# BOpermanis/SP-SLAM

Measured on AMD Instinct MI355X. Metric: RGB-D frames/sec (track+planes+poseOpt) at 640x480; ATE vs CPU ref, higher is better.
Workload: dtype u8+f32+f64

## Files before the change

### include/spslam_gpu.h

```cpp
#ifndef SPSLAM_GPU_H
#define SPSLAM_GPU_H

#include <stddef.h>
#include <stdint.h>

#ifdef __cplusplus
extern "C" {
#endif

#define SPSLAM_OK 0
#define SPSLAM_ERR_ARG (-1)
#define SPSLAM_ERR_CAPACITY (-2)
#define SPSLAM_ERR_HIP (-3)
#define SPSLAM_ERR_NOT_READY (-4)

typedef struct spslam_ctx spslam_ctx;

typedef struct spslam_keypoint {
    float x, y;
    float size;
    float angle;
    float response;
    int32_t octave;
    int32_t class_id;
// ... 232 lines not shown
int spslam_supposed_debug(spslam_ctx* ctx, int frame, int plane, spslam_line_candidate* cand, int* n_cand,
                          int32_t* idx, int idx_cap);

int spslam_planes_debug(spslam_ctx* ctx, int frame, int what, void* out, int* n_points);

int spslam_debug_plane_labels(spslam_ctx* ctx, int keep);

typedef struct spslam_plane_launch_shape {
    int32_t seg_maps_in_lds;
    int32_t seg_positions;
    int32_t wave_count;
    int32_t one_workgroup;
    int32_t barrier_rows;
} spslam_plane_launch_shape;
int spslam_debug_plane_launch_shape(spslam_ctx* ctx, int n_frames, spslam_plane_launch_shape* shape);

int spslam_debug_plane_not_seen(spslam_ctx* ctx, const float* planes, int n_planes, const float* coefs, int n_coefs,
                                int* not_seen);

int spslam_debug_libm64(spslam_ctx* ctx, int kind, const double* a, const double* b, int n, double* out);

int spslam_debug_pose_spin_cap(spslam_ctx* ctx, int cap);

int spslam_debug_force_solve_failures(spslam_ctx* ctx, unsigned trial_mask);

#define SPSLAM_GRID_COLS 64
#define SPSLAM_GRID_ROWS 48

typedef struct spslam_frame_params {
    float fx, fy, cx, cy;
// ... 495 lines not shown
```

### sp-slam_amd/csrc/capi_planes.cpp

```cpp
#include "capi_ctx.h"

#include <cmath>
#include <cstring>
#include <random>
#include <string>

namespace {

hipError_t configure_supposed(spslam_ctx* c, const spslam_plane_params* p) {
    const PlaneGeom& g = c->pg;
    SuppParams& sp = c->sp;
    sp.line_ratio = p->line_ratio;
    const double T = (double)p->line_distance_threshold * (double)p->line_distance_threshold;
    float f = (float)T;
    while ((double)f >= T && f > 0.f) f = std::nextafter(f, 0.f);
    while ((double)std::nextafter(f, 1.f) < T) f = std::nextafter(f, 1.f);
    sp.sqr_th_f = f;
    const bool nob = p->image_bounds[0] == 0.f && p->image_bounds[1] == 0.f && p->image_bounds[2] == 0.f &&
                     p->image_bounds[3] == 0.f;
    sp.min_x = nob ? 0.f : p->image_bounds[0];
    sp.max_x = nob ? (float)p->width : p->image_bounds[1];
    sp.min_y = nob ? 0.f : p->image_bounds[2];
    sp.max_y = nob ? (float)p->height : p->image_bounds[3];
    sp.supp_cap = kMaxSuppPerFrame;
    sp.line_cap = g.contour_cap;
    int ns = 0;
    for (float v = -0.25f; v < 0.25f; v = (float)((double)v + 0.01)) {
        if (ns >= kMaxPatchSteps) return hipErrorInvalidValue;
        sp.steps[ns++] = v;
    }
    sp.n_steps = ns;
    const size_t F = (size_t)c->p.max_batch, CC = (size_t)g.contour_cap;
    SuppBuffers& b = c->sb;
    const size_t bytes = (size_t)kSuppRndTable * 4 +
                         F * kMaxPlanesPerFrame * kMaxLinesPerBoundary * sizeof(LineCand) +
                         F * kMaxPlanesPerFrame * sizeof(int) + F * CC * (4 + 16 + 4 + 1) +
                         F * kMaxPlanesPerFrame * 8 * sizeof(long long) + 9 * 256;
    hipError_t e = c->d_supp_scratch.alloc(bytes);
    if (e != hipSuccess) return e;
    uint8_t* q = c->d_supp_scratch;
    auto carve = [&](size_t n) { uint8_t* r = q; q += (n + 255) / 256 * 256; return r; };
    b.rnd = (const uint32_t*)carve((size_t)kSuppRndTable * 4);
    b.cand = (LineCand*)carve(F * kMaxPlanesPerFrame * kMaxLinesPerBoundary * sizeof(LineCand));
    b.n_cand = (int*)carve(F * kMaxPlanesPerFrame * sizeof(int));
    b.line_idx = (int32_t*)carve(F * CC * 4);
    b.big = (float4*)carve(F * CC * 16);
    b.big_sh = (int*)carve(F * CC * 4);
    b.big_flag = (uint8_t*)carve(F * CC);
    b.prof = (long long*)carve(F * kMaxPlanesPerFrame * 8 * sizeof(long long));
    e = hipMemset(b.prof, 0, F * kMaxPlanesPerFrame * 8 * sizeof(long long));
    if (e != hipSuccess) return e;
    std::vector<uint32_t> tab(kSuppRndTable);
    std::mt19937 mt(12345u);
    for (auto& v : tab) v = (uint32_t)mt() >> 1;
    e = hipMemcpy((void*)b.rnd, tab.data(), tab.size() * 4, hipMemcpyHostToDevice);
    if (e != hipSuccess) return e;
    const size_t patch = (size_t)sp.n_steps * sp.n_steps;
    if ((e = c->d_supp1.alloc(sp.supp_cap * sizeof(spslam_supposed_plane))) != hipSuccess) return e;
    if ((e = c->d_supp_cnt1.alloc(16)) != hipSuccess) return e;
    if ((e = c->d_line1.alloc(CC * 4)) != hipSuccess) return e;
    return c->d_patch1.alloc(sp.supp_cap * patch * 12);
}

int plane_status_flags(long long word, int epoch) { return (word >> 8) == epoch ? (int)(word & 0xFF) : 0; }

}

extern "C" {

int spslam_planes_configure(spslam_ctx* c, const spslam_plane_params* p) {
// ... 15 lines not shown
    if (plane_launch_shape(g, 1, nullptr) != hipSuccess)
        return fail(c, SPSLAM_ERR_ARG, "no kernel instance takes the organized cloud%s",
                    g.W > 512 ? ": wider than 512 columns" : ": past the segmentation's LDS or index budget");
    g.fx = p->fx; g.fy = p->fy; g.cx = p->cx; g.cy = p->cy;
    g.min_size = p->min_size;
    g.ang_cos = std::cos((float)(0.017453 * p->angle_threshold));
    g.dist_th = p->distance_threshold;
    g.inlier_cap = g.N;
    g.contour_cap = 4 * g.N;
    c->pg = g;
    const long long N = g.N, F = c->p.max_batch, IWH = (long long)(g.W + 1) * (g.H + 1);
    PlaneBuffers& b = c->pb;
    c->planes_ready = false;
    c->plane_last_frames = c->supp_last_frames = 0;
    c->plane_cloud[0] = c->plane_cloud[1] = nullptr;
    c->sb = SuppBuffers{};
    const int keep_labels = b.keep_labels;
    b = PlaneBuffers{};
    b.keep_labels = keep_labels;
    const long long SH = wave_size(g.W, g.H);
    b.cloud_fs = 3 * N; b.wave_fs = SH; b.dist_fs = N; b.integral_fs = 6 * (IWH + g.W + 1); b.normal_fs = 3 * N; b.pd_fs = N;
    b.labels_fs = N; b.work_fs = 4 * N; b.grown_fs = N; b.maps_fs = 2 * N;
    const size_t bytes = F * (sizeof(float) * (2 * b.cloud_fs + b.wave_fs + b.dist_fs + b.normal_fs + b.pd_fs) +
                              sizeof(double) * b.integral_fs + sizeof(uint32_t) * b.labels_fs +
                              sizeof(int) * (b.work_fs + b.grown_fs) + b.maps_fs + 16 * sizeof(long long)) + 8192;
    HIP_CHECK(c, c->d_plane_scratch.alloc(bytes));
    uint8_t* q = c->d_plane_scratch;
    auto carve = [&](size_t n) { uint8_t* r = q; q += (n + 255) / 256 * 256; return r; };
    b.integral = (double*)carve(F * b.integral_fs * sizeof(double));
    c->plane_cloud[0] = (float*)carve(F * b.cloud_fs * 4);
    c->plane_cloud[1] = (float*)carve(F * b.cloud_fs * 4);
// ... 264 lines not shown
        return rc;
    HIP_CHECK(c, plane_not_seen_debug_launch(st.slot<float>(0), n_planes, st.slot<float>(1), n_coefs,
                                             st.slot<int>(2), c->stream));
    HIP_CHECK(c, hipMemcpyAsync(not_seen, st.slot<int>(2), (size_t)n_coefs * 4, hipMemcpyDeviceToHost, c->stream));
    if (int rc = st.close()) return rc;
    HIP_CHECK(c, hipStreamSynchronize(c->stream));
    return SPSLAM_OK;
}

int spslam_debug_plane_labels(spslam_ctx* c, int keep) {
    if (!c) return SPSLAM_ERR_ARG;
    c->pb.keep_labels = keep ? 1 : 0;
    return SPSLAM_OK;
}

int spslam_supposed_debug(spslam_ctx* c, int frame, int plane, spslam_line_candidate* cand, int* n_cand,
                          int32_t* idx, int idx_cap) {
    static_assert(sizeof(spslam_line_candidate) == sizeof(LineCand), "candidate layout");
    if (!c || !cand || !n_cand) return SPSLAM_ERR_ARG;
    if (frame < 0 || frame >= c->supp_last_frames || plane < 0 || plane >= kMaxPlanesPerFrame)
        return fail(c, SPSLAM_ERR_NOT_READY, "no supposed-plane data for that frame%s", "");
    HIP_CHECK(c, hipSetDevice(c->device));
    HIP_CHECK(c, hipDeviceSynchronize());
    int nc = 0;
    HIP_CHECK(c, hipMemcpy(&nc, c->sb.n_cand + frame * kMaxPlanesPerFrame + plane, sizeof(int), hipMemcpyDeviceToHost));
    nc = std::min(std::max(nc, 0), kMaxLinesPerBoundary);
    LineCand lc[kMaxLinesPerBoundary];
    if (nc)
        HIP_CHECK(c, hipMemcpy(lc, c->sb.cand + ((size_t)frame * kMaxPlanesPerFrame + plane) * kMaxLinesPerBoundary,
                               nc * sizeof(LineCand), hipMemcpyDeviceToHost));
// ... 61 lines not shown
```

### sp-slam_amd/csrc/supposed_kernels.hip

```cpp
#include "pcl_eigen33.h"
#include "plane_not_seen.h"
#include "supposed_launch.h"
#include "wave_ops.h"

namespace spslam {
namespace supp {

using namespace pcl_eigen;

constexpr int kThreads = 256, kWaves = 4;
constexpr int kMaxWaves = 8;
constexpr int kBatch = 64;
constexpr int kLdsPts = 2048;
constexpr int kMaxTrials = 1001;

#ifdef SPSLAM_SUPP_PROF
#define SUPP_CLK() ((long long)__builtin_amdgcn_s_memrealtime())
#define SUPP_T(k) do { if (t == 0) { const long long c_ = SUPP_CLK(); pr[k] += c_ - pt; pt = c_; } } while (0)
#else
#define SUPP_T(k) do { } while (0)
#endif

struct Shared {
    int s0[kBatch], s1[kBatch], cnt[kBatch];
    int nb, fail, done, have;
    int iterations, best, best_s0, best_s1;
    double k;
    float line[6];
    float acc[9];
    int red[kMaxWaves];
    int n_inl, flags;
    int s0x[kBatch], s1x[kBatch], nbb[2], failb[2];
};

template <int NT>
__device__ int block_sum(int v, Shared& S) {
    const int lane = threadIdx.x & 63, wave = threadIdx.x >> 6;
    v = wave_sum(v);
    __syncthreads();
    if (lane == 0) S.red[wave] = v;
    __syncthreads();
    int s = 0;
#pragma unroll
    for (int w = 0; w < NT / 64; w++) s += S.red[w];
    return s;
}

// ... 103 lines not shown
}

template <int NT>
__device__ int select_within(const float* coef, const float4* Q, uint8_t* flag, int n, float thr, Shared& S) {
    float lp[3] = {coef[0], coef[1], coef[2]}, ld[3] = {coef[3], coef[4], coef[5]};
    normalize4(ld);
    int c = 0;
    for (int i = threadIdx.x; i < n; i += NT) {
        const bool in = line_sqd(lp, ld, Q[i]) <= thr;
        flag[i] = in;
        c += in;
    }
    return block_sum<NT>(c, S);
}

#ifndef SPSLAM_SUPP_OVERLAP
#define SPSLAM_SUPP_OVERLAP 1
#endif
#ifndef SPSLAM_SUPP_OVERLAP_ALL
#define SPSLAM_SUPP_OVERLAP_ALL 0
#endif
#ifndef SPSLAM_SUPP_MINB
#define SPSLAM_SUPP_MINB 3
#endif
template <int NT>
__global__ __launch_bounds__(NT, NT == 256 ? SPSLAM_SUPP_MINB : 1) void supp_lines_kernel(PlaneGeom g, PlaneBuffers pb, SuppParams sp,
                                                              SuppBuffers sb, const float* __restrict__ depth,
                                                              long long depth_fs, int depth_stride,
                                                              const spslam_plane* __restrict__ planes,
                                                              const int* __restrict__ plane_counts,
                                                              const int32_t* __restrict__ contours) {
    __shared__ float4 Qs[kLdsPts];
    __shared__ int shs[kLdsPts];
    __shared__ uint8_t flags_s[kLdsPts];
#ifdef SPSLAM_MEASURE_SKIP_SUPP
    if (g.W > 0) return;
#endif
    __shared__ Shared S;
    constexpr bool kOverlap = SPSLAM_SUPP_OVERLAP && (NT == 512 || SPSLAM_SUPP_OVERLAP_ALL);
    const int f = blockIdx.x, t = threadIdx.x, lane = t & 63, wave = t >> 6;
    const int np = min(plane_counts[f], kMaxPlanesPerFrame);
    const spslam_plane* P = planes + (size_t)f * kMaxPlanesPerFrame;
    const int32_t* con = contours + (size_t)f * g.contour_cap;
    const float* X = pb.cloud + f * pb.cloud_fs;
    const float* Y = X + g.N;
    const float* Z = X + 2 * g.N;
    const Cam K{g.fx, g.fy, g.cx, g.cy, sp.min_x, sp.max_x, sp.min_y, sp.max_y, g.w, g.h, depth_stride};
    const float* D = depth + f * depth_fs;
    const float thr = sp.sqr_th_f;
    for (int q = blockIdx.y; q < np; q += gridDim.y) {
        LineCand* C = sb.cand + ((size_t)f * kMaxPlanesPerFrame + q) * kMaxLinesPerBoundary;
        const int bsize = P[q].n_contour, coff = P[q].contour_offset;
        if (bsize < 50) {
            if (t == 0) sb.n_cand[f * kMaxPlanesPerFrame + q] = 0;
            continue;
        }
        const bool in_lds = bsize <= kLdsPts;
        int32_t* lidx = sb.line_idx + (size_t)f * g.contour_cap + coff;
        auto boundary = [&](float4* Q, int* sh, uint8_t* flag) __attribute__((always_inline)) -> int {
#ifdef SPSLAM_SUPP_PROF
        long long pr[8] = {0, 0, 0, 0, 0, 0, 0, 0}, pt = SUPP_CLK();
#endif
        for (int i = t; i < bsize; i += NT) {
            const int ci = con[coff + i];
            Q[i] = make_float4(X[ci], Y[ci], Z[ci], __int_as_float(ci));
        }
        __syncthreads();
        SUPP_T(0);
        int n = bsize, used = 0, ncand = 0;
        for (int j = 0; j < kMaxLinesPerBoundary; j++) {
            if (t == 0) {
                S.iterations = 0; S.best = -2147483647; S.k = 1.0; S.have = 0; S.done = n < 2;
            }
            if constexpr (kOverlap) {
                if (t < kBatch) S.cnt[t] = 0;
            }
            for (int i = t; i < n; i += NT) sh[i] = i;
            __syncthreads();
            const double one_over_n = 1.0 / (double)n, log_prob = log(1.0 - 0.99);
            int r0 = 0, r1 = 1;
            uint32_t pos = 0;
            int bp0 = 0, bp1 = 0, qh = 0, qn = 0;
            uint64_t gmask = 0;
            uint32_t rnext = wave == 0 ? sb.rnd[lane] : 0u;
            if constexpr (!kOverlap) {
                while (!S.done) {
                    if (wave == 0) {
                        const int it0 = S.iterations;
                        int nb = 0, chk = 0;
                        bool fail = false;
                        while (nb < kBatch && it0 + nb < kMaxTrials) {
                            if (qh == qn) {
                                const uint32_t r = rnext;
                                const uint32_t jv = (lane & 1) ? 1u + r % (uint32_t)(n - 1) : r % (uint32_t)n;
                                pos += 64;
                                rnext = sb.rnd[pos + lane];
    #pragma unroll 4
                                for (int c = 0; c < 32; c++) {
                                    const int j0 = __builtin_amdgcn_readlane((int)jv, 2 * c), j1 = __builtin_amdgcn_readlane((int)jv, 2 * c + 1);
                                    const int i0 = j0 > 1 ? j0 : 0, i1 = j1 > 1 ? j1 : 1;
                                    const int x0 = sh[i0], x1 = sh[i1];
                                    const int a0 = r0, b0 = r1;
                                    const int r1m = j0 == 1 ? a0 : b0;
                                    sh[i0] = a0;
                                    sh[i1] = r1m;
                                    r0 = j0 > 1 ? x0 : (j0 == 1 ? b0 : a0);
                                    r1 = j1 > 1 ? (j1 == j0 ? a0 : x1) : r1m;
                                    bp0 = lane == c ? r0 : bp0;
                                    bp1 = lane == c ? r1 : bp1;
                                }
                                bool good = false;
                                if (lane < 32) {
                                    const float4 a = Q[bp0], b = Q[bp1];
                                    good = a.x != b.x && a.y != b.y && a.z != b.z;
                                }
                                gmask = __ballot(good);
                                qh = 0;
                                qn = 32;
                            }
                            const uint64_t m = gmask & (~0ull << qh) & 0xFFFFFFFFull;
                            if (m == 0) {
                                chk += qn - qh;
                                qh = qn;
                                if (chk >= 1000) { fail = true; break; }
                                continue;
                            }
                            const int gi = __ffsll((unsigned long long)m) - 1;
                            if (chk + (gi - qh) >= 1000) { fail = true; break; }
                            const int s0v = __builtin_amdgcn_readlane(bp0, gi), s1v = __builtin_amdgcn_readlane(bp1, gi);
                            if (lane == 0) { S.s0[nb] = s0v; S.s1[nb] = s1v; }
                            nb++;
                            chk = 0;
                            qh = gi + 1;
                        }
                        if (lane == 0) { S.nb = nb; S.fail = fail; }
                    }
                    __syncthreads();
                    SUPP_T(1);
                    const int nb = S.nb;
                    {
                        constexpr int NW = NT / 64;
                        const int c = wave * (kBatch / NW) + lane / NW, qq = lane % NW;
                        int cnt = 0;
                        if (c < nb) {
                            float L[6];
                            line_from_samples(Q[S.s0[c]], Q[S.s1[c]], L);
                            float ld[3] = {L[3], L[4], L[5]};
                            normalize4(ld);
    #pragma unroll 1
                            for (int i = qq; i < n; i += NW) cnt += line_sqd(L, ld, Q[i]) <= thr;
                        }
    #pragma unroll
                        for (int o = 1; o < NW; o <<= 1) cnt += __shfl_xor(cnt, o);
                        if (qq == 0 && c < nb) S.cnt[c] = cnt;
                    }
                    __syncthreads();
                    SUPP_T(2);
                    if (wave == 0) {
                        const int it0 = S.iterations, best0 = S.best;
                        const double k0 = S.k;
                        const bool act = lane < nb;
                        const int cn = act ? S.cnt[lane] : INT_MIN;
                        int pm = cn, lr;
    #pragma unroll
                        for (int off = 1; off < 64; off <<= 1) {
                            const int y = __shfl_up(pm, off);
                            if (lane >= off) pm = max(pm, y);
                        }
                        int ex = __shfl_up(pm, 1);
                        if (lane == 0) ex = INT_MIN;
                        const bool rec = act && cn > max(ex, best0);
                        double kc = 0.0;
                        if (rec) {
                            const double w = (double)cn * one_over_n;
                            double pno = 1.0 - w * w;
                            pno = fmax(DBL_EPSILON, pno);
                            pno = fmin(1.0 - DBL_EPSILON, pno);
                            kc = log_prob / log(pno);
                        }
                        lr = rec ? lane : -1;
    #pragma unroll
                        for (int off = 1; off < 64; off <<= 1) {
                            const int y = __shfl_up(lr, off);
                            if (lane >= off) lr = max(lr, y);
                        }
                        int lre = __shfl_up(lr, 1);
                        if (lane == 0) lre = -1;
                        const double kb_rec = __shfl(kc, lre < 0 ? 0 : lre);
                        const double kb = lre < 0 ? k0 : kb_rec;
                        const uint64_t m1 = __ballot(act && !((double)(it0 + lane) < kb));
                        const int stop1 = m1 ? __ffsll((unsigned long long)m1) - 1 : 64;
                        const int stop2 = (kMaxTrials - 1) - it0;
                        int proc, it;
                        bool done;
                        if (stop1 < nb && stop1 <= stop2) { proc = stop1; it = it0 + stop1; done = true; }
                        else if (stop2 < nb) { proc = stop2 + 1; it = it0 + stop2 + 1; done = true; }
                        else { proc = nb; it = it0 + nb; done = false; }
                        const uint64_t rm = __ballot(rec) & (proc >= 64 ? ~0ull : ((1ull << proc) - 1ull));
                        double kf = k0;
                        if (rm) {
                            const int L = 63 - __clzll(rm);
                            kf = __shfl(kc, L);
                            if (lane == L) {
                                S.best = cn; S.best_s0 = S.s0[L]; S.best_s1 = S.s1[L]; S.have = 1; S.k = kc;
                            }
                        }
                        if (!done && (S.fail || !((double)it < kf))) done = true;
                        if (lane == 0) {
                            S.iterations = it;
                            S.done = done;
                        }
                    }
                    __syncthreads();
                    SUPP_T(3);
    #ifdef SPSLAM_SUPP_PROF
                    if (t == 0) pr[6]++;
    #endif
                }
            } else {
                auto sample = [&](int sb_, int it0) __attribute__((always_inline)) {
                    int nb = 0, chk = 0;
                    bool fail = false;
                    while (nb < kBatch && it0 + nb < kMaxTrials) {
                        if (qh == qn) {
                            const uint32_t r = rnext;
                            const uint32_t jv = (lane & 1) ? 1u + r % (uint32_t)(n - 1) : r % (uint32_t)n;
                            pos += 64;
                            rnext = sb.rnd[pos + lane];
    #pragma unroll 4
                            for (int c = 0; c < 32; c++) {
                                const int j0 = __builtin_amdgcn_readlane((int)jv, 2 * c), j1 = __builtin_amdgcn_readlane((int)jv, 2 * c + 1);
                                const int i0 = j0 > 1 ? j0 : 0, i1 = j1 > 1 ? j1 : 1;
                                const int x0 = sh[i0], x1 = sh[i1];
                                const int a0 = r0, b0 = r1;
                                const int r1m = j0 == 1 ? a0 : b0;
                                sh[i0] = a0;
                                sh[i1] = r1m;
                                r0 = j0 > 1 ? x0 : (j0 == 1 ? b0 : a0);
                                r1 = j1 > 1 ? (j1 == j0 ? a0 : x1) : r1m;
                                bp0 = lane == c ? r0 : bp0;
                                bp1 = lane == c ? r1 : bp1;
                            }
                            bool good = false;
                            if (lane < 32) {
                                const float4 a = Q[bp0], b = Q[bp1];
                                good = a.x != b.x && a.y != b.y && a.z != b.z;
                            }
                            gmask = __ballot(good);
                            qh = 0;
                            qn = 32;
                        }
                        const uint64_t m = gmask & (~0ull << qh) & 0xFFFFFFFFull;
                        if (m == 0) {
                            chk += qn - qh;
                            qh = qn;
                            if (chk >= 1000) { fail = true; break; }
                            continue;
                        }
                        const int gi = __ffsll((unsigned long long)m) - 1;
                        if (chk + (gi - qh) >= 1000) { fail = true; break; }
                        const int s0v = __builtin_amdgcn_readlane(bp0, gi), s1v = __builtin_amdgcn_readlane(bp1, gi);
                        if (lane == 0) { (sb_ ? S.s0x : S.s0)[nb] = s0v; (sb_ ? S.s1x : S.s1)[nb] = s1v; }
                        nb++;
                        chk = 0;
                        qh = gi + 1;
                    }
                    if (lane == 0) { S.nbb[sb_] = nb; S.failb[sb_] = fail; }
                };
                auto decide = [&](int sb_, int nb) __attribute__((always_inline)) {
                    const int it0 = S.iterations, best0 = S.best;
                    const double k0 = S.k;
                    const bool act = lane < nb;
                    const int cn = act ? S.cnt[lane] : INT_MIN;
                    int pm = cn, lr;
    #pragma unroll
                    for (int off = 1; off < 64; off <<= 1) {
                        const int y = __shfl_up(pm, off);
                        if (lane >= off) pm = max(pm, y);
                    }
                    int ex = __shfl_up(pm, 1);
                    if (lane == 0) ex = INT_MIN;
                    const bool rec = act && cn > max(ex, best0);
                    double kc = 0.0;
                    if (rec) {
                        const double w = (double)cn * one_over_n;
                        double pno = 1.0 - w * w;
                        pno = fmax(DBL_EPSILON, pno);
                        pno = fmin(1.0 - DBL_EPSILON, pno);
                        kc = log_prob / log(pno);
                    }
                    lr = rec ? lane : -1;
    #pragma unroll
                    for (int off = 1; off < 64; off <<= 1) {
                        const int y = __shfl_up(lr, off);
                        if (lane >= off) lr = max(lr, y);
                    }
                    int lre = __shfl_up(lr, 1);
                    if (lane == 0) lre = -1;
                    const double kb_rec = __shfl(kc, lre < 0 ? 0 : lre);
                    const double kb = lre < 0 ? k0 : kb_rec;
                    const uint64_t m1 = __ballot(act && !((double)(it0 + lane) < kb));
                    const int stop1 = m1 ? __ffsll((unsigned long long)m1) - 1 : 64;
                    const int stop2 = (kMaxTrials - 1) - it0;
                    int proc, it;
                    bool done;
                    if (stop1 < nb && stop1 <= stop2) { proc = stop1; it = it0 + stop1; done = true; }
                    else if (stop2 < nb) { proc = stop2 + 1; it = it0 + stop2 + 1; done = true; }
                    else { proc = nb; it = it0 + nb; done = false; }
                    const uint64_t rm = __ballot(rec) & (proc >= 64 ? ~0ull : ((1ull << proc) - 1ull));
                    double kf = k0;
                    if (rm) {
                        const int L = 63 - __clzll(rm);
                        kf = __shfl(kc, L);
                        if (lane == L) {
                            S.best = cn; S.best_s0 = (sb_ ? S.s0x : S.s0)[L]; S.best_s1 = (sb_ ? S.s1x : S.s1)[L];
                            S.have = 1; S.k = kc;
                        }
                    }
                    if (!done && (S.failb[sb_] || !((double)it < kf))) done = true;
                    if (lane == 0) {
                        S.iterations = it;
                        S.done = done;
                    }
                };
                if (wave == 0 && !S.done) sample(0, 0);
                __syncthreads();
                SUPP_T(1);
                int cur = 0;
                while (!S.done) {
                    const int nb = S.nbb[cur];
                    if (wave == 0) {
                        if (!S.failb[cur]) sample(cur ^ 1, S.iterations + nb);
                        else if (lane == 0) { S.nbb[cur ^ 1] = 0; S.failb[cur ^ 1] = 1; }
                    } else {
                        constexpr int LP = NT / 64 - 1;
                        const int u = t - 64, c = u / LP, qq = u - c * LP;
                        if (c < nb) {
                            float L[6];
                            line_from_samples(Q[(cur ? S.s0x : S.s0)[c]], Q[(cur ? S.s1x : S.s1)[c]], L);
                            float ld[3] = {L[3], L[4], L[5]};
                            normalize4(ld);
                            int cnt = 0;
#pragma unroll 1
                            for (int i = qq; i < n; i += LP) cnt += line_sqd(L, ld, Q[i]) <= thr;
                            atomicAdd(&S.cnt[c], cnt);
                        }
                    }
                    __syncthreads();
                    SUPP_T(2);
                    if (wave == 0) {
                        decide(cur, nb);
                        S.cnt[lane] = 0;
                    }
                    __syncthreads();
                    SUPP_T(3);
#ifdef SPSLAM_SUPP_PROF
                    if (t == 0) pr[6]++;
#endif
                    cur ^= 1;
                }
            }
            int n_inl = 0;
            if (S.have) {
                float c0[6];
                line_from_samples(Q[S.best_s0], Q[S.best_s1], c0);
                n_inl = select_within<NT>(c0, Q, flag, n, thr, S);
                if (n_inl > 2) {
                    constexpr int kG = 8;
                    if (wave == 0 && lane < 3) {
                        float s = 0.f;
                        int i = 0;
                        for (; i + kG <= n; i += kG) {
                            float v[kG];
#pragma unroll
                            for (int u = 0; u < kG; u++) {
                                const float4 p = Q[i + u];
                                v[u] = flag[i + u] ? (lane == 0 ? p.x : lane == 1 ? p.y : p.z) : 0.f;
                            }
#pragma unroll
                            for (int u = 0; u < kG; u++) s += v[u];
                        }
                        for (; i < n; i++) {
                            const float4 p = Q[i];
                            s += flag[i] ? (lane == 0 ? p.x : lane == 1 ? p.y : p.z) : 0.f;
                        }
                        S.acc[lane] = s / (float)n_inl;
                    }
                    __syncthreads();
                    if (wave == 0 && lane < 6) {
                        const float cx = S.acc[0], cy = S.acc[1], cz = S.acc[2];
                        auto term = [&](int i) __attribute__((always_inline)) {
                            const float4 p = Q[i];
                            const float x = p.x - cx, y = p.y - cy, z = p.z - cz;
                            const float a = lane == 0 ? y : lane == 1 ? y : lane == 2 ? z : lane == 3 ? x : lane == 4 ? y : z;
                            const float b = lane == 0 ? y : lane == 1 ? z : lane == 2 ? z : x;
                            return flag[i] ? a * b : 0.f;
                        };
                        float s = 0.f;
                        int i = 0;
                        for (; i + kG <= n; i += kG) {
                            float v[kG];
#pragma unroll
                            for (int u = 0; u < kG; u++) v[u] = term(i + u);
#pragma unroll
                            for (int u = 0; u < kG; u++) s += v[u];
                        }
                        for (; i < n; i++) s += term(i);
                        S.acc[3 + lane] = s;
                    }
                    __syncthreads();
                    if (t == 0) {
                        const float cov[3][3] = {{S.acc[6], S.acc[7], S.acc[8]},
                                                 {S.acc[7], S.acc[3], S.acc[4]},
                                                 {S.acc[8], S.acc[4], S.acc[5]}};
                        float ev[3];
                        line_direction(cov, ev);
                        S.line[0] = S.acc[0]; S.line[1] = S.acc[1]; S.line[2] = S.acc[2];
                        S.line[3] = ev[0]; S.line[4] = ev[1]; S.line[5] = ev[2];
                    }
                } else if (t == 0) {
                    for (int k = 0; k < 6; k++) S.line[k] = c0[k];
                }
// ... 51 lines not shown
            nonborder = block_sum<NT>(nonborder, S);
            if (t == 0) out.flags = fl | ((fl & 2) && nonborder <= n_inl / 4 ? 4 : 0);
            used += n_inl;
            n = kbase;
            __syncthreads();
            SUPP_T(5);
        }
#ifdef SPSLAM_SUPP_PROF
        if (t == 0) {
            pr[7] = bsize;
            for (int k = 0; k < 8; k++) sb.prof[((size_t)f * kMaxPlanesPerFrame + q) * 8 + k] = pr[k];
        }
#endif
            return ncand;
        };
        const int ncand = in_lds ? boundary(Qs, shs, flags_s)
                                 : boundary(sb.big + (size_t)f * g.contour_cap + coff,
                                            sb.big_sh + (size_t)f * g.contour_cap + coff,
                                            sb.big_flag + (size_t)f * g.contour_cap + coff);
        if (t == 0) sb.n_cand[f * kMaxPlanesPerFrame + q] = ncand;
        __syncthreads();
    }
}

__device__ void supposed_coef(const float* ip, const float* il, float* coef) {
    const float a = fmaf(ip[1], il[5], -(ip[2] * il[4]));
    const float b = fmaf(ip[2], il[3], -(ip[0] * il[5]));
    const float c = fmaf(ip[0], il[4], -(ip[1] * il[3]));
    const float d = fmaf(c, il[2], fmaf(a, il[0], b * il[1]));
    const float v = sqrtf(fmaf(c, c, fmaf(a, a, b * b)));
    coef[0] = a / v; coef[1] = b / v; coef[2] = c / v; coef[3] = -d / v;
    if (coef[3] < 0)
        for (int k = 0; k < 4; k++) coef[k] = -coef[k];
}
// ... 118 lines not shown
```

### sp-slam_amd/csrc/supposed_launch.h

```cpp
#pragma once
#include <hip/hip_runtime.h>

#include "../../include/spslam_gpu.h"
#include "orb_launch.h"
#include "plane_launch.h"

namespace spslam {

constexpr int kMaxLinesPerBoundary = 4;
constexpr int kSuppRndTable = 1 << 21;
constexpr int kMaxPatchSteps = 64;
constexpr int kMaxSuppPerFrame = 32;

struct LineCand {
    float line[6];
    int n_inliers;
    int iterations;
    int flags;
    int idx_off;
};

struct SuppParams {
    double line_ratio;
    float sqr_th_f;
    float min_x, max_x, min_y, max_y;
    int supp_cap;
    int line_cap;
    int n_steps;
    float steps[kMaxPatchSteps];
};

struct SuppBuffers {
    const uint32_t* rnd;
    LineCand* cand;
    int* n_cand;
    int32_t* line_idx;
    float4* big;
    int* big_sh;
    uint8_t* big_flag;
    long long* prof;
};

hipError_t supp_launch(const PlaneGeom& g, const PlaneBuffers& pb, const SuppParams& sp, const SuppBuffers& sb,
                       int n, const float* depth, long long depth_fs, int depth_stride, const spslam_plane* planes,
                       const int* plane_counts, const int32_t* contours, spslam_supposed_plane* out, int* out_counts,
                       int32_t* out_line_idx, float* out_patch, hipStream_t s, KernelTimer* timer);

hipError_t plane_not_seen_debug_launch(const float* planes, int n, const float* coefs, int m, int* out,
// ... 4 lines not shown
```

### sp-slam_amd/spslam_planes.py

```python
from __future__ import annotations

import ctypes

import numpy as np

import spslam_gpu

PLANE_DTYPE = np.dtype([("coef", "<f4", 4), ("n_inliers", "<i4"), ("inlier_offset", "<i4"), ("n_contour", "<i4"),
                        ("contour_offset", "<i4")])
assert PLANE_DTYPE.itemsize == 32


class PlaneParams(ctypes.Structure):
    _fields_ = [("cloud_dis", ctypes.c_int), ("min_size", ctypes.c_int), ("angle_threshold", ctypes.c_float),
                ("distance_threshold", ctypes.c_float), ("fx", ctypes.c_float), ("fy", ctypes.c_float),
                ("cx", ctypes.c_float), ("cy", ctypes.c_float), ("width", ctypes.c_int), ("height", ctypes.c_int),
                ("line_ratio", ctypes.c_double), ("line_distance_threshold", ctypes.c_float),
                ("image_bounds", ctypes.c_float * 4)]


SUPPOSED_DTYPE = np.dtype([("coef", "<f4", 4), ("line", "<f4", 6), ("source_plane", "<i4"), ("n_line", "<i4"),
                           ("line_offset", "<i4"), ("n_patch", "<i4"), ("patch_offset", "<i4"), ("pad", "<i4")])
assert SUPPOSED_DTYPE.itemsize == 64
LINE_CAND_DTYPE = np.dtype([("line", "<f4", 6), ("n_inliers", "<i4"), ("iterations", "<i4"), ("flags", "<i4"),
                            ("idx_offset", "<i4")])


spslam_gpu.EXPORTED += ["spslam_planes_configure", "spslam_planes_capacity", "spslam_planes_extract",
                        "spslam_planes_extract_batch_device", "spslam_planes_debug", "spslam_debug_plane_labels",
                        "spslam_supposed_capacity",
                        "spslam_planes_generate_from_boundaries",
                        "spslam_planes_generate_from_boundaries_batch_device", "spslam_supposed_debug",
                        "spslam_planes_select_cloud_set",
                        "spslam_debug_plane_not_seen", "spslam_planes_status", "spslam_debug_plane_launch_shape"]

OVER_COMPONENTS, OVER_MODELS, OVER_KEPT = 1, 2, 4


class PlaneLaunchShape(ctypes.Structure):
    _fields_ = [("seg_maps_in_lds", ctypes.c_int32), ("seg_positions", ctypes.c_int32),
                ("wave_count", ctypes.c_int32), ("one_workgroup", ctypes.c_int32), ("barrier_rows", ctypes.c_int32)]


def _bind(lib):
    vp, ip = ctypes.c_void_p, ctypes.POINTER(ctypes.c_int)
    lib.spslam_planes_configure.argtypes = [vp, ctypes.POINTER(PlaneParams)]
    lib.spslam_planes_capacity.argtypes = [vp, ip, ip, ip]
    lib.spslam_planes_extract.argtypes = [vp, vp, ctypes.c_int, ctypes.c_int, ctypes.c_int, vp, ctypes.c_int, ip, vp,
                                          vp]
# ... 77 lines not shown

    def status(self, frame=0):
        flags = ctypes.c_int(-1)
        self.ex._check(self.ex.lib.spslam_planes_status(self.ex.ctx, frame, ctypes.byref(flags)))
        return flags.value

    def launch_shape(self, n_frames=1):
        sh = PlaneLaunchShape()
        self.ex._check(self.ex.lib.spslam_debug_plane_launch_shape(self.ex.ctx, n_frames, ctypes.byref(sh)))
        return {name: int(getattr(sh, name)) for name, _ in PlaneLaunchShape._fields_}

    def keep_labels(self, on=True):
        self.ex.lib.spslam_debug_plane_labels.argtypes = [ctypes.c_void_p, ctypes.c_int]
        self.ex._check(self.ex.lib.spslam_debug_plane_labels(self.ex.ctx, int(on)))

    def debug(self, frame, what):
        N = self.W * self.H
        shape, dt = {0: ((N, 3), np.float32), 1: ((N, 3), np.float32), 2: (N, np.float32), 3: (N, np.uint32)}[what]
        out = np.zeros(shape, dt)
        n = ctypes.c_int()
        self.ex._check(self.ex.lib.spslam_planes_debug(self.ex.ctx, frame, what, out.ctypes.data, ctypes.byref(n)))
        return out

    def generate_from_boundaries(self, depth_f32: np.ndarray):
        d = np.ascontiguousarray(depth_f32, np.float32)
        out = np.zeros(self.supp_cap, SUPPOSED_DTYPE)
        lines = np.zeros(self.line_cap, np.int32)
        patch = np.zeros((self.supp_cap * self.patch_points, 3), np.float32)
        n = ctypes.c_int()
        self.ex._check(self.ex.lib.spslam_planes_generate_from_boundaries(
# ... 34 lines not shown
```

Before: 44550.

## Precompute RANSAC sample-pair table per point count and compact inliers for line refit

```diff
diff --git a/include/spslam_gpu.h b/include/spslam_gpu.h
--- a/include/spslam_gpu.h
+++ b/include/spslam_gpu.h
@@ -270,6 +270,10 @@
     int32_t barrier_rows;
 } spslam_plane_launch_shape;
 int spslam_debug_plane_launch_shape(spslam_ctx* ctx, int n_frames, spslam_plane_launch_shape* shape);
+
+int spslam_debug_supposed_table_depth(spslam_ctx* ctx, int pairs);
+
+int spslam_debug_supposed_table_row(spslam_ctx* ctx, int n, uint32_t* pairs);
 
 int spslam_debug_plane_not_seen(spslam_ctx* ctx, const float* planes, int n_planes, const float* coefs, int n_coefs,
                                 int* not_seen);
diff --git a/sp-slam_amd/csrc/capi_planes.cpp b/sp-slam_amd/csrc/capi_planes.cpp
--- a/sp-slam_amd/csrc/capi_planes.cpp
+++ b/sp-slam_amd/csrc/capi_planes.cpp
@@ -32,15 +32,17 @@
     sp.n_steps = ns;
     const size_t F = (size_t)c->p.max_batch, CC = (size_t)g.contour_cap;
     SuppBuffers& b = c->sb;
-    const size_t bytes = (size_t)kSuppRndTable * 4 +
+    const size_t n_samples = supp_sample_row(kSuppTabMaxN + 1);
+    const size_t bytes = (size_t)kSuppRndTable * 4 + n_samples * 4 +
                          F * kMaxPlanesPerFrame * kMaxLinesPerBoundary * sizeof(LineCand) +
                          F * kMaxPlanesPerFrame * sizeof(int) + F * CC * (4 + 16 + 4 + 1) +
-                         F * kMaxPlanesPerFrame * 8 * sizeof(long long) + 9 * 256;
+                         F * kMaxPlanesPerFrame * 8 * sizeof(long long) + 10 * 256;
     hipError_t e = c->d_supp_scratch.alloc(bytes);
     if (e != hipSuccess) return e;
     uint8_t* q = c->d_supp_scratch;
     auto carve = [&](size_t n) { uint8_t* r = q; q += (n + 255) / 256 * 256; return r; };
     b.rnd = (const uint32_t*)carve((size_t)kSuppRndTable * 4);
+    b.samples = (const uint32_t*)carve(n_samples * 4);
     b.cand = (LineCand*)carve(F * kMaxPlanesPerFrame * kMaxLinesPerBoundary * sizeof(LineCand));
     b.n_cand = (int*)carve(F * kMaxPlanesPerFrame * sizeof(int));
     b.line_idx = (int32_t*)carve(F * CC * 4);
@@ -54,6 +56,9 @@
     std::mt19937 mt(12345u);
     for (auto& v : tab) v = (uint32_t)mt() >> 1;
     e = hipMemcpy((void*)b.rnd, tab.data(), tab.size() * 4, hipMemcpyHostToDevice);
+    if (e != hipSuccess) return e;
+    const std::vector<uint32_t> samples = build_supp_sample_table(tab.data());
+    e = hipMemcpy((void*)b.samples, samples.data(), samples.size() * 4, hipMemcpyHostToDevice);
     if (e != hipSuccess) return e;
     const size_t patch = (size_t)sp.n_steps * sp.n_steps;
     if ((e = c->d_supp1.alloc(sp.supp_cap * sizeof(spslam_supposed_plane))) != hipSuccess) return e;
@@ -99,7 +104,9 @@
     c->planes_ready = false;
     c->plane_last_frames = c->supp_last_frames = 0;
     c->plane_cloud[0] = c->plane_cloud[1] = nullptr;
+    const int tab_depth = c->sb.tab_depth;
     c->sb = SuppBuffers{};
+    c->sb.tab_depth = tab_depth;
     const int keep_labels = b.keep_labels;
     b = PlaneBuffers{};
     b.keep_labels = keep_labels;
@@ -394,6 +401,20 @@
     return SPSLAM_OK;
 }
 
+int spslam_debug_supposed_table_depth(spslam_ctx* c, int pairs) {
+    if (!c || pairs < 0 || pairs > kSuppTabPairs) return SPSLAM_ERR_ARG;
+    c->sb.tab_depth = pairs;
+    return SPSLAM_OK;
+}
+
+int spslam_debug_supposed_table_row(spslam_ctx* c, int n, uint32_t* pairs) {
+    if (!c || !pairs || n < kSuppTabMinN || n > kSuppTabMaxN) return SPSLAM_ERR_ARG;
+    if (!c->planes_ready) return fail(c, SPSLAM_ERR_NOT_READY, "spslam_planes_configure not called%s", "");
+    HIP_CHECK(c, hipSetDevice(c->device));
+    HIP_CHECK(c, hipMemcpy(pairs, c->sb.samples + supp_sample_row(n), kSuppTabPairs * 4, hipMemcpyDeviceToHost));
+    return SPSLAM_OK;
+}
+
 int spslam_supposed_debug(spslam_ctx* c, int frame, int plane, spslam_line_candidate* cand, int* n_cand,
                           int32_t* idx, int idx_cap) {
     static_assert(sizeof(spslam_line_candidate) == sizeof(LineCand), "candidate layout");
diff --git a/sp-slam_amd/csrc/supp_sample_table.h b/sp-slam_amd/csrc/supp_sample_table.h
--- /dev/null
+++ b/sp-slam_amd/csrc/supp_sample_table.h
@@ -0,0 +1,29 @@
+#pragma once
+#include <cstddef>
+#include <cstdint>
+#include <vector>
+
+namespace spslam {
+
+constexpr int kSuppTabMinN = 2, kSuppTabMaxN = 2048;
+constexpr int kSuppTabPairs = 1024;
+
+constexpr size_t supp_sample_row(int n) { return (size_t)(n - kSuppTabMinN) * kSuppTabPairs; }
+
+inline std::vector<uint32_t> build_supp_sample_table(const uint32_t* draws) {
+    std::vector<uint32_t> tab((size_t)(kSuppTabMaxN - kSuppTabMinN + 1) * kSuppTabPairs);
+    std::vector<uint16_t> sh(kSuppTabMaxN);
+    for (int n = kSuppTabMinN; n <= kSuppTabMaxN; n++) {
+        for (int i = 0; i < n; i++) sh[i] = (uint16_t)i;
+        uint32_t* row = tab.data() + supp_sample_row(n);
+        for (int k = 0; k < kSuppTabPairs; k++) {
+            const uint32_t j0 = draws[2 * k] % (uint32_t)n, j1 = 1u + draws[2 * k + 1] % (uint32_t)(n - 1);
+            uint16_t x = sh[0]; sh[0] = sh[j0]; sh[j0] = x;
+            x = sh[1]; sh[1] = sh[j1]; sh[j1] = x;
+            row[k] = (uint32_t)sh[0] | (uint32_t)sh[1] << 16;
+        }
+    }
+    return tab;
+}
+
+}
diff --git a/sp-slam_amd/csrc/supposed_kernels.hip b/sp-slam_amd/csrc/supposed_kernels.hip
--- a/sp-slam_amd/csrc/supposed_kernels.hip
+++ b/sp-slam_amd/csrc/supposed_kernels.hip
@@ -13,6 +13,7 @@
 constexpr int kBatch = 64;
 constexpr int kLdsPts = 2048;
 constexpr int kMaxTrials = 1001;
+static_assert(kSuppTabMaxN == kLdsPts, "the sample table has a row for every point count of an LDS boundary");
 
 #ifdef SPSLAM_SUPP_PROF
 #define SUPP_CLK() ((long long)__builtin_amdgcn_s_memrealtime())
@@ -30,7 +31,6 @@
     float acc[9];
     int red[kMaxWaves];
     int n_inl, flags;
-    int s0x[kBatch], s1x[kBatch], nbb[2], failb[2];
 };
 
 template <int NT>
@@ -164,12 +164,29 @@
     return block_sum<NT>(c, S);
 }
 
-#ifndef SPSLAM_SUPP_OVERLAP
-#define SPSLAM_SUPP_OVERLAP 1
-#endif
-#ifndef SPSLAM_SUPP_OVERLAP_ALL
-#define SPSLAM_SUPP_OVERLAP_ALL 0
-#endif
+template <int NT>
+__device__ void compact_flagged(const uint8_t* flag, int* list, int n, Shared& S) {
+    const int lane = threadIdx.x & 63, wave = threadIdx.x >> 6;
+    const uint64_t lt = (lane == 0) ? 0ull : (~0ull >> (64 - lane));
+    int base = 0;
+    for (int b0 = 0; b0 < n; b0 += NT) {
+        const int i = b0 + (int)threadIdx.x;
+        const bool in = i < n && flag[i];
+        const uint64_t m = __ballot(in);
+        if (lane == 0) S.cnt[wave] = __popcll(m);
+        __syncthreads();
+        int o = base;
+#pragma unroll
+        for (int w = 0; w < NT / 64; w++) {
+            const int c = S.cnt[w];
+            o += w < wave ? c : 0;
+            base += c;
+        }
+        if (in) list[o + __popcll(m & lt)] = i;
+        __syncthreads();
+    }
+}
+
 #ifndef SPSLAM_SUPP_MINB
 #define SPSLAM_SUPP_MINB 3
 #endif
@@ -187,7 +204,6 @@
     if (g.W > 0) return;
 #endif
     __shared__ Shared S;
-    constexpr bool kOverlap = SPSLAM_SUPP_OVERLAP && (NT == 512 || SPSLAM_SUPP_OVERLAP_ALL);
     const int f = blockIdx.x, t = threadIdx.x, lane = t & 63, wave = t >> 6;
     const int np = min(plane_counts[f], kMaxPlanesPerFrame);
     const spslam_plane* P = planes + (size_t)f * kMaxPlanesPerFrame;
@@ -207,7 +223,7 @@
         }
         const bool in_lds = bsize <= kLdsPts;
         int32_t* lidx = sb.line_idx + (size_t)f * g.contour_cap + coff;
-        auto boundary = [&](float4* Q, int* sh, uint8_t* flag) __attribute__((always_inline)) -> int {
+        auto boundary = [&](float4* Q, int* sh, uint8_t* flag, const bool tab) __attribute__((always_inline)) -> int {
 #ifdef SPSLAM_SUPP_PROF
         long long pr[8] = {0, 0, 0, 0, 0, 0, 0, 0}, pt = SUPP_CLK();
 #endif
@@ -222,185 +238,76 @@
             if (t == 0) {
                 S.iterations = 0; S.best = -2147483647; S.k = 1.0; S.have = 0; S.done = n < 2;
             }
-            if constexpr (kOverlap) {
-                if (t < kBatch) S.cnt[t] = 0;
-            }
-            for (int i = t; i < n; i += NT) sh[i] = i;
+            if (!tab)
+                for (int i = t; i < n; i += NT) sh[i] = i;
             __syncthreads();
             const double one_over_n = 1.0 / (double)n, log_prob = log(1.0 - 0.99);
+            const int depth = tab ? sb.tab_depth : 0;
+            const uint32_t* trow = sb.samples + supp_sample_row(n < kSuppTabMinN ? kSuppTabMinN : n);
+            bool live = !tab;
+            int tp = 0;
             int r0 = 0, r1 = 1;
             uint32_t pos = 0;
             int bp0 = 0, bp1 = 0, qh = 0, qn = 0;
             uint64_t gmask = 0;
-            uint32_t rnext = wave == 0 ? sb.rnd[lane] : 0u;
-            if constexpr (!kOverlap) {
-                while (!S.done) {
-                    if (wave == 0) {
-                        const int it0 = S.iterations;
-                        int nb = 0, chk = 0;
-                        bool fail = false;
-                        while (nb < kBatch && it0 + nb < kMaxTrials) {
-                            if (qh == qn) {
-                                const uint32_t r = rnext;
-                                const uint32_t jv = (lane & 1) ? 1u + r % (uint32_t)(n - 1) : r % (uint32_t)n;
-                                pos += 64;
-                                rnext = sb.rnd[pos + lane];
-    #pragma unroll 4
-                                for (int c = 0; c < 32; c++) {
-                                    const int j0 = __builtin_amdgcn_readlane((int)jv, 2 * c), j1 = __builtin_amdgcn_readlane((int)jv, 2 * c + 1);
-                                    const int i0 = j0 > 1 ? j0 : 0, i1 = j1 > 1 ? j1 : 1;
-                                    const int x0 = sh[i0], x1 = sh[i1];
-                                    const int a0 = r0, b0 = r1;
-                                    const int r1m = j0 == 1 ? a0 : b0;
-                                    sh[i0] = a0;
-                                    sh[i1] = r1m;
-                                    r0 = j0 > 1 ? x0 : (j0 == 1 ? b0 : a0);
-                                    r1 = j1 > 1 ? (j1 == j0 ? a0 : x1) : r1m;
-                                    bp0 = lane == c ? r0 : bp0;
-                                    bp1 = lane == c ? r1 : bp1;
+            uint32_t rnext = 0u;
+            if (wave == 0) rnext = !tab ? sb.rnd[lane] : (n >= kSuppTabMinN && lane < depth) ? trow[lane] : 0u;
+            auto chain = [&](const int m) __attribute__((always_inline)) {
+                const uint32_t r = rnext;
+                const uint32_t jv = (lane & 1) ? 1u + r % (uint32_t)(n - 1) : r % (uint32_t)n;
+                pos += 2 * m;
+                rnext = sb.rnd[pos + lane];
+#pragma unroll 4
+                for (int c = 0; c < 32; c++) {
+                    if (c >= m) continue;
+                    const int j0 = __builtin_amdgcn_readlane((int)jv, 2 * c), j1 = __builtin_amdgcn_readlane((int)jv, 2 * c + 1);
+                    const int i0 = j0 > 1 ? j0 : 0, i1 = j1 > 1 ? j1 : 1;
+                    const int x0 = sh[i0], x1 = sh[i1];
+                    const int a0 = r0, b0 = r1;
+                    const int r1m = j0 == 1 ? a0 : b0;
+                    sh[i0] = a0;
+                    sh[i1] = r1m;
+                    r0 = j0 > 1 ? x0 : (j0 == 1 ? b0 : a0);
+                    r1 = j1 > 1 ? (j1 == j0 ? a0 : x1) : r1m;
+                    bp0 = lane == c ? r0 : bp0;
+                    bp1 = lane == c ? r1 : bp1;
+                }
+            };
+            while (!S.done) {
+                if (wave == 0) {
+                    const int it0 = S.iterations;
+                    const int want = min(kBatch, kMaxTrials - it0);
+                    int nb = 0, chk = 0;
+                    bool fail = false;
+                    while (nb < want) {
+                        if (qh == qn) {
+                            if (!live && tp < depth) {
+                                const uint32_t e = rnext;
+                                qn = min(64, depth - tp);
+                                tp += 64;
+                                rnext = tp + lane < depth ? trow[tp + lane] : 0u;
+                                bp0 = (int)(e & 0xFFFFu);
+                                bp1 = (int)(e >> 16);
+                            } else {
+                                if (!live) {
+                                    live = true;
+                                    for (int i = lane; i < n; i += 64) sh[i] = i;
+                                    wave_sync();
+                                    rnext = sb.rnd[lane];
+                                    for (int left = depth; left > 0; left -= 32) chain(min(32, left));
                                 }
-                                bool good = false;
-                                if (lane < 32) {
-                                    const float4 a = Q[bp0], b = Q[bp1];
-                                    good = a.x != b.x && a.y != b.y && a.z != b.z;
-                                }
-                                gmask = __ballot(good);
-                                qh = 0;
+                                chain(32);
                                 qn = 32;
                             }
-                            const uint64_t m = gmask & (~0ull << qh) & 0xFFFFFFFFull;
-                            if (m == 0) {
-                                chk += qn - qh;
-                                qh = qn;
-                                if (chk >= 1000) { fail = true; break; }
-                                continue;
-                            }
-                            const int gi = __ffsll((unsigned long long)m) - 1;
-                            if (chk + (gi - qh) >= 1000) { fail = true; break; }
-                            const int s0v = __builtin_amdgcn_readlane(bp0, gi), s1v = __builtin_amdgcn_readlane(bp1, gi);
-                            if (lane == 0) { S.s0[nb] = s0v; S.s1[nb] = s1v; }
-                            nb++;
-                            chk = 0;
-                            qh = gi + 1;
-                        }
-                        if (lane == 0) { S.nb = nb; S.fail = fail; }
-                    }
-                    __syncthreads();
-                    SUPP_T(1);
-                    const int nb = S.nb;
-                    {
-                        constexpr int NW = NT / 64;
-                        const int c = wave * (kBatch / NW) + lane / NW, qq = lane % NW;
-                        int cnt = 0;
-                        if (c < nb) {
-                            float L[6];
-                            line_from_samples(Q[S.s0[c]], Q[S.s1[c]], L);
-                            float ld[3] = {L[3], L[4], L[5]};
-                            normalize4(ld);
-    #pragma unroll 1
-                            for (int i = qq; i < n; i += NW) cnt += line_sqd(L, ld, Q[i]) <= thr;
-                        }
-    #pragma unroll
-                        for (int o = 1; o < NW; o <<= 1) cnt += __shfl_xor(cnt, o);
-                        if (qq == 0 && c < nb) S.cnt[c] = cnt;
-                    }
-                    __syncthreads();
-                    SUPP_T(2);
-                    if (wave == 0) {
-                        const int it0 = S.iterations, best0 = S.best;
-                        const double k0 = S.k;
-                        const bool act = lane < nb;
-                        const int cn = act ? S.cnt[lane] : INT_MIN;
-                        int pm = cn, lr;
-    #pragma unroll
-                        for (int off = 1; off < 64; off <<= 1) {
-                            const int y = __shfl_up(pm, off);
-                            if (lane >= off) pm = max(pm, y);
-                        }
-                        int ex = __shfl_up(pm, 1);
-                        if (lane == 0) ex = INT_MIN;
-                        const bool rec = act && cn > max(ex, best0);
-                        double kc = 0.0;
-                        if (rec) {
-                            const double w = (double)cn * one_over_n;
-                            double pno = 1.0 - w * w;
-                            pno = fmax(DBL_EPSILON, pno);
-                            pno = fmin(1.0 - DBL_EPSILON, pno);
-                            kc = log_prob / log(pno);
-                        }
-                        lr = rec ? lane : -1;
-    #pragma unroll
-                        for (int off = 1; off < 64; off <<= 1) {
-                            const int y = __shfl_up(lr, off);
-                            if (lane >= off) lr = max(lr, y);
-                        }
-                        int lre = __shfl_up(lr, 1);
-                        if (lane == 0) lre = -1;
-                        const double kb_rec = __shfl(kc, lre < 0 ? 0 : lre);
-                        const double kb = lre < 0 ? k0 : kb_rec;
-                        const uint64_t m1 = __ballot(act && !((double)(it0 + lane) < kb));
-                        const int stop1 = m1 ? __ffsll((unsigned long long)m1) - 1 : 64;
-                        const int stop2 = (kMaxTrials - 1) - it0;
-                        int proc, it;
-                        bool done;
-                        if (stop1 < nb && stop1 <= stop2) { proc = stop1; it = it0 + stop1; done = true; }
-                        else if (stop2 < nb) { proc = stop2 + 1; it = it0 + stop2 + 1; done = true; }
-                        else { proc = nb; it = it0 + nb; done = false; }
-                        const uint64_t rm = __ballot(rec) & (proc >= 64 ? ~0ull : ((1ull << proc) - 1ull));
-                        double kf = k0;
-                        if (rm) {
-                            const int L = 63 - __clzll(rm);
-                            kf = __shfl(kc, L);
-                            if (lane == L) {
-                                S.best = cn; S.best_s0 = S.s0[L]; S.best_s1 = S.s1[L]; S.have = 1; S.k = kc;
-                            }
-                        }
-                        if (!done && (S.fail || !((double)it < kf))) done = true;
-                        if (lane == 0) {
-                            S.iterations = it;
-                            S.done = done;
-                        }
-                    }
-                    __syncthreads();
-                    SUPP_T(3);
-    #ifdef SPSLAM_SUPP_PROF
-                    if (t == 0) pr[6]++;
-    #endif
-                }
-            } else {
-                auto sample = [&](int sb_, int it0) __attribute__((always_inline)) {
-                    int nb = 0, chk = 0;
-                    bool fail = false;
-                    while (nb < kBatch && it0 + nb < kMaxTrials) {
-                        if (qh == qn) {
-                            const uint32_t r = rnext;
-                            const uint32_t jv = (lane & 1) ? 1u + r % (uint32_t)(n - 1) : r % (uint32_t)n;
-                            pos += 64;
-                            rnext = sb.rnd[pos + lane];
-    #pragma unroll 4
-                            for (int c = 0; c < 32; c++) {
-                                const int j0 = __builtin_amdgcn_readlane((int)jv, 2 * c), j1 = __builtin_amdgcn_readlane((int)jv, 2 * c + 1);
-                                const int i0 = j0 > 1 ? j0 : 0, i1 = j1 > 1 ? j1 : 1;
-                                const int x0 = sh[i0], x1 = sh[i1];
-                                const int a0 = r0, b0 = r1;
-                                const int r1m = j0 == 1 ? a0 : b0;
-                                sh[i0] = a0;
-                                sh[i1] = r1m;
-                                r0 = j0 > 1 ? x0 : (j0 == 1 ? b0 : a0);
-                                r1 = j1 > 1 ? (j1 == j0 ? a0 : x1) : r1m;
-                                bp0 = lane == c ? r0 : bp0;
-                                bp1 = lane == c ? r1 : bp1;
-                            }
                             bool good = false;
-                            if (lane < 32) {
+                            if (lane < qn) {
                                 const float4 a = Q[bp0], b = Q[bp1];
                                 good = a.x != b.x && a.y != b.y && a.z != b.z;
                             }
                             gmask = __ballot(good);
                             qh = 0;
-                            qn = 32;
                         }
-                        const uint64_t m = gmask & (~0ull << qh) & 0xFFFFFFFFull;
+                        const uint64_t m = gmask & (~0ull << qh);
                         if (m == 0) {
                             chk += qn - qh;
                             qh = qn;
@@ -409,21 +316,45 @@
                         }
                         const int gi = __ffsll((unsigned long long)m) - 1;
                         if (chk + (gi - qh) >= 1000) { fail = true; break; }
-                        const int s0v = __builtin_amdgcn_readlane(bp0, gi), s1v = __builtin_amdgcn_readlane(bp1, gi);
-                        if (lane == 0) { (sb_ ? S.s0x : S.s0)[nb] = s0v; (sb_ ? S.s1x : S.s1)[nb] = s1v; }
-                        nb++;
+                        const int take = min(__popcll(m), want - nb);
+                        const int rank = (int)__builtin_amdgcn_mbcnt_hi((uint32_t)(m >> 32), __builtin_amdgcn_mbcnt_lo((uint32_t)m, 0u));
+                        const bool mine = ((m >> lane) & 1ull) && rank < take;
+                        if (mine) { S.s0[nb + rank] = bp0; S.s1[nb + rank] = bp1; }
+                        const uint64_t lastm = __ballot(mine && rank == take - 1);
+                        nb += take;
                         chk = 0;
-                        qh = gi + 1;
-                    }
-                    if (lane == 0) { S.nbb[sb_] = nb; S.failb[sb_] = fail; }
-                };
-                auto decide = [&](int sb_, int nb) __attribute__((always_inline)) {
+                        qh = __ffsll((unsigned long long)lastm);
+                    }
+                    if (lane == 0) { S.nb = nb; S.fail = fail; }
+                }
+                __syncthreads();
+                SUPP_T(1);
+                const int nb = S.nb;
+                {
+                    constexpr int NW = NT / 64;
+                    const int c = wave * (kBatch / NW) + lane / NW, qq = lane % NW;
+                    int cnt = 0;
+                    if (c < nb) {
+                        float L[6];
+                        line_from_samples(Q[S.s0[c]], Q[S.s1[c]], L);
+                        float ld[3] = {L[3], L[4], L[5]};
+                        normalize4(ld);
+#pragma unroll 1
+                        for (int i = qq; i < n; i += NW) cnt += line_sqd(L, ld, Q[i]) <= thr;
+                    }
+#pragma unroll
+                    for (int o = 1; o < NW; o <<= 1) cnt += __shfl_xor(cnt, o);
+                    if (qq == 0 && c < nb) S.cnt[c] = cnt;
+                }
+                __syncthreads();
+                SUPP_T(2);
+                if (wave == 0) {
                     const int it0 = S.iterations, best0 = S.best;
                     const double k0 = S.k;
                     const bool act = lane < nb;
                     const int cn = act ? S.cnt[lane] : INT_MIN;
                     int pm = cn, lr;
-    #pragma unroll
+#pragma unroll
                     for (int off = 1; off < 64; off <<= 1) {
                         const int y = __shfl_up(pm, off);
                         if (lane >= off) pm = max(pm, y);
@@ -440,7 +371,7 @@
                         kc = log_prob / log(pno);
                     }
                     lr = rec ? lane : -1;
-    #pragma unroll
+#pragma unroll
                     for (int off = 1; off < 64; off <<= 1) {
                         const int y = __shfl_up(lr, off);
                         if (lane >= off) lr = max(lr, y);
@@ -463,52 +394,20 @@
                         const int L = 63 - __clzll(rm);
                         kf = __shfl(kc, L);
                         if (lane == L) {
-                            S.best = cn; S.best_s0 = (sb_ ? S.s0x : S.s0)[L]; S.best_s1 = (sb_ ? S.s1x : S.s1)[L];
-                            S.have = 1; S.k = kc;
+                            S.best = cn; S.best_s0 = S.s0[L]; S.best_s1 = S.s1[L]; S.have = 1; S.k = kc;
                         }
                     }
-                    if (!done && (S.failb[sb_] || !((double)it < kf))) done = true;
+                    if (!done && (S.fail || !((double)it < kf))) done = true;
                     if (lane == 0) {
                         S.iterations = it;
                         S.done = done;
                     }
-                };
-                if (wave == 0 && !S.done) sample(0, 0);
+                }
                 __syncthreads();
-                SUPP_T(1);
-                int cur = 0;
-                while (!S.done) {
-                    const int nb = S.nbb[cur];
-                    if (wave == 0) {
-                        if (!S.failb[cur]) sample(cur ^ 1, S.iterations + nb);
-                        else if (lane == 0) { S.nbb[cur ^ 1] = 0; S.failb[cur ^ 1] = 1; }
-                    } else {
-                        constexpr int LP = NT / 64 - 1;
-                        const int u = t - 64, c = u / LP, qq = u - c * LP;
-                        if (c < nb) {
-                            float L[6];
-                            line_from_samples(Q[(cur ? S.s0x : S.s0)[c]], Q[(cur ? S.s1x : S.s1)[c]], L);
-                            float ld[3] = {L[3], L[4], L[5]};
-                            normalize4(ld);
-                            int cnt = 0;
-#pragma unroll 1
-                            for (int i = qq; i < n; i += LP) cnt += line_sqd(L, ld, Q[i]) <= thr;
-                            atomicAdd(&S.cnt[c], cnt);
-                        }
-                    }
-                    __syncthreads();
-                    SUPP_T(2);
-                    if (wave == 0) {
-                        decide(cur, nb);
-                        S.cnt[lane] = 0;
-                    }
-                    __syncthreads();
-                    SUPP_T(3);
+                SUPP_T(3);
 #ifdef SPSLAM_SUPP_PROF
-                    if (t == 0) pr[6]++;
+                if (t == 0) pr[6]++;
 #endif
-                    cur ^= 1;
-                }
             }
             int n_inl = 0;
             if (S.have) {
@@ -516,46 +415,45 @@
                 line_from_samples(Q[S.best_s0], Q[S.best_s1], c0);
                 n_inl = select_within<NT>(c0, Q, flag, n, thr, S);
                 if (n_inl > 2) {
+                    compact_flagged<NT>(flag, sh, n, S);
                     constexpr int kG = 8;
                     if (wave == 0 && lane < 3) {
+                        auto term = [&](int k) __attribute__((always_inline)) {
+                            const float4 p = Q[sh[k]];
+                            return lane == 0 ? p.x : lane == 1 ? p.y : p.z;
+                        };
                         float s = 0.f;
                         int i = 0;
-                        for (; i + kG <= n; i += kG) {
+                        for (; i + kG <= n_inl; i += kG) {
                             float v[kG];
 #pragma unroll
-                            for (int u = 0; u < kG; u++) {
-                                const float4 p = Q[i + u];
-                                v[u] = flag[i + u] ? (lane == 0 ? p.x : lane == 1 ? p.y : p.z) : 0.f;
-                            }
+                            for (int u = 0; u < kG; u++) v[u] = term(i + u);
 #pragma unroll
                             for (int u = 0; u < kG; u++) s += v[u];
                         }
-                        for (; i < n; i++) {
-                            const float4 p = Q[i];
-                            s += flag[i] ? (lane == 0 ? p.x : lane == 1 ? p.y : p.z) : 0.f;
-                        }
+                        for (; i < n_inl; i++) s += term(i);
                         S.acc[lane] = s / (float)n_inl;
                     }
                     __syncthreads();
                     if (wave == 0 && lane < 6) {
                         const float cx = S.acc[0], cy = S.acc[1], cz = S.acc[2];
-                        auto term = [&](int i) __attribute__((always_inline)) {
-                            const float4 p = Q[i];
+                        auto term = [&](int k) __attribute__((always_inline)) {
+                            const float4 p = Q[sh[k]];
                             const float x = p.x - cx, y = p.y - cy, z = p.z - cz;
                             const float a = lane == 0 ? y : lane == 1 ? y : lane == 2 ? z : lane == 3 ? x : lane == 4 ? y : z;
                             const float b = lane == 0 ? y : lane == 1 ? z : lane == 2 ? z : x;
-                            return flag[i] ? a * b : 0.f;
+                            return a * b;
                         };
                         float s = 0.f;
                         int i = 0;
-                        for (; i + kG <= n; i += kG) {
+                        for (; i + kG <= n_inl; i += kG) {
                             float v[kG];
 #pragma unroll
                             for (int u = 0; u < kG; u++) v[u] = term(i + u);
 #pragma unroll
                             for (int u = 0; u < kG; u++) s += v[u];
                         }
-                        for (; i < n; i++) s += term(i);
+                        for (; i < n_inl; i++) s += term(i);
                         S.acc[3 + lane] = s;
                     }
                     __syncthreads();
@@ -637,10 +535,10 @@
 #endif
             return ncand;
         };
-        const int ncand = in_lds ? boundary(Qs, shs, flags_s)
+        const int ncand = in_lds ? boundary(Qs, shs, flags_s, true)
                                  : boundary(sb.big + (size_t)f * g.contour_cap + coff,
                                             sb.big_sh + (size_t)f * g.contour_cap + coff,
-                                            sb.big_flag + (size_t)f * g.contour_cap + coff);
+                                            sb.big_flag + (size_t)f * g.contour_cap + coff, false);
         if (t == 0) sb.n_cand[f * kMaxPlanesPerFrame + q] = ncand;
         __syncthreads();
     }
diff --git a/sp-slam_amd/csrc/supposed_launch.h b/sp-slam_amd/csrc/supposed_launch.h
--- a/sp-slam_amd/csrc/supposed_launch.h
+++ b/sp-slam_amd/csrc/supposed_launch.h
@@ -4,6 +4,7 @@
 #include "../../include/spslam_gpu.h"
 #include "orb_launch.h"
 #include "plane_launch.h"
+#include "supp_sample_table.h"
 
 namespace spslam {
 
@@ -32,6 +33,8 @@
 
 struct SuppBuffers {
     const uint32_t* rnd;
+    const uint32_t* samples;
+    int tab_depth = kSuppTabPairs;
     LineCand* cand;
     int* n_cand;
     int32_t* line_idx;
diff --git a/sp-slam_amd/spslam_planes.py b/sp-slam_amd/spslam_planes.py
--- a/sp-slam_amd/spslam_planes.py
+++ b/sp-slam_amd/spslam_planes.py
@@ -32,7 +32,8 @@
                         "spslam_planes_generate_from_boundaries",
                         "spslam_planes_generate_from_boundaries_batch_device", "spslam_supposed_debug",
                         "spslam_planes_select_cloud_set",
-                        "spslam_debug_plane_not_seen", "spslam_planes_status", "spslam_debug_plane_launch_shape"]
+                        "spslam_debug_plane_not_seen", "spslam_planes_status", "spslam_debug_plane_launch_shape",
+                        "spslam_debug_supposed_table_depth", "spslam_debug_supposed_table_row"]
 
 OVER_COMPONENTS, OVER_MODELS, OVER_KEPT = 1, 2, 4
 
@@ -140,6 +141,18 @@
         self.ex.lib.spslam_debug_plane_labels.argtypes = [ctypes.c_void_p, ctypes.c_int]
         self.ex._check(self.ex.lib.spslam_debug_plane_labels(self.ex.ctx, int(on)))
 
+    SAMPLE_TABLE_PAIRS = 1024
+
+    def supposed_table_depth(self, pairs=SAMPLE_TABLE_PAIRS):
+        self.ex.lib.spslam_debug_supposed_table_depth.argtypes = [ctypes.c_void_p, ctypes.c_int]
+        self.ex._check(self.ex.lib.spslam_debug_supposed_table_depth(self.ex.ctx, int(pairs)))
+
+    def supposed_table_row(self, n):
+        row = np.zeros(self.SAMPLE_TABLE_PAIRS, np.uint32)
+        self.ex.lib.spslam_debug_supposed_table_row.argtypes = [ctypes.c_void_p, ctypes.c_int, ctypes.c_void_p]
+        self.ex._check(self.ex.lib.spslam_debug_supposed_table_row(self.ex.ctx, int(n), row.ctypes.data))
+        return np.stack([row & 0xFFFF, row >> 16], 1).astype(np.int64)
+
     def debug(self, frame, what):
         N = self.W * self.H
         shape, dt = {0: ((N, 3), np.float32), 1: ((N, 3), np.float32), 2: (N, np.float32), 3: (N, np.uint32)}[what]
```

After: 44460 (median of 2 runs). About the same (-0.2%).
